# arun-sub/genomicsbench

Hardware: AMD Instinct MI355X
Metric: bsw_large_gcups (higher is better)
Workload: dtype int32

## Files before the change

genomicsbench_amd/csrc/bsw_kernels.hip:

```cpp
#include "gbx_internal.h"
#include <atomic>
#include <climits>
#include <cstdlib>

namespace gbx {
namespace {

constexpr int NEG = -(1 << 29);
constexpr int BIGJ = 1 << 20;

constexpr int NCLS = 21;
constexpr int CLS_LDS = NCLS - 1;
constexpr int NTB = 32;
constexpr int NBIN = NCLS * NTB;
constexpr int HDR = 1024;
constexpr int REG_SCORE_LIMIT = 1 << 20;

struct BswDev {
    int o_del, e_del, o_ins, e_ins, oe_del, oe_ins, zdrop, end_bonus, w, max_mat;
    uint32_t colword[5];
    int32_t col4[5];
    uint32_t row0[5];
    uint32_t row1[5];
    uint8_t remap[24];
// ... 325 lines not shown
            zm |= nz << c;
        }
        Hs[CPL] = 0;

        const int key = group_allmax<LPP>(((kl >> 5) << KB) | (j0 + (kl & 31)));
        const int m = key >> KB, mj = key & ((1 << KB) - 1);
        const int zf_l = zm ? j0 + (__builtin_ffs((int)zm) - 1) : BIGJ;
        const int zl_l = zm ? j0 + (31 - __builtin_clz(zm)) : -1;
        const int zfirst = BIGJ - group_allmax<LPP>(BIGJ - zf_l);
        const int zlast = group_allmax<LPP>(zl_l);

        const bool live = b < e;
        const int jfin = live ? e : b;
        const int hend = live ? hl : left0;
        const bool gq = jfin == qlen;
        g_i = (gq & (hend >= g_score)) ? i : g_i;
        g_score = gq ? max(g_score, hend) : g_score;
        const bool upd = (m > best) & (m != 0);
        const int dd = (i - best_i) - (mj - best_j);
        const int pen = max(__mul24(dd, e_del), __mul24(-dd, e_ins));
        const bool zbrk = (prm.zdrop > 0) & !upd & (best - m - pen > prm.zdrop);
        const bool brk = (m == 0) | zbrk;
        const int dmi = mj - i;
        off = upd ? imax3(off, dmi, -dmi) : off;
        best_i = upd ? i : best_i;
        best_j = upd ? mj : best_j;
        best = upd ? m : best;
        beg = min(zfirst, e);
        end = min(zlast + 2, qlen);
        ++i;
        done = active & (brk | (i >= tlen));
    }
}

__global__ void __launch_bounds__(64) bsw_lds_kernel(BswDev prm, BswPairs P, BswWork W, int cls)
{
    extern __shared__ int lds[];
    const int lane = threadIdx.x;
    const int first = W.base[cls * NTB];
    const int cnt = W.base[(cls + 1) * NTB] - first;
    const int32_t *order = W.order + first;
    const int e_ins = prm.e_ins, e_del = prm.e_del, oe_ins = prm.oe_ins, oe_del = prm.oe_del;

    for (int slot = blockIdx.x; slot < cnt; slot += gridDim.x) {
        const int pair = order[slot];
        const int qlen = P.len2[pair], tlen = P.len1[pair], h0 = P.h0[pair];
        const uint8_t *q = P.qer + P.idq[pair];
        const uint8_t *tp = P.ref + P.idr[pair];
        int *hd = lds, *ev = lds + (qlen + 1);
        for (int j = lane; j <= qlen; j += 64) {
            hd[j] = j == 0 ? h0 : max(h0 - oe_ins - (j - 1) * e_ins, 0);
            ev[j] = 0;
        }
        __syncthreads();
        int w;
        {
            int lim = (int)((double)(qlen * prm.max_mat + prm.end_bonus - prm.o_ins) / (double)e_ins + 1.);
            lim = max(lim, 1); w = min(prm.w, lim);
            lim = (int)((double)(qlen * prm.max_mat + prm.end_bonus - prm.o_del) / (double)e_del + 1.);
            lim = max(lim, 1); w = min(w, lim);
        }
        int best = h0, best_i = -1, best_j = -1, g_i = -1, g_score = -1, off = 0;
        int beg = 0, end = qlen;
        for (int i = 0; i < tlen; ++i) {
            const int b = max(beg, i - w);
            const int e = min(min(end, i + w + 1), qlen);
            const int left0 = b == 0 ? max(h0 - (prm.o_del + e_del * (i + 1)), 0) : 0;
            const int t = min((int)tp[i], 4);
            int fcarry = NEG;
            int left = left0;
            int m = 0, mj = -1;
            int zfirst = BIGJ, zlast = -1;
            if (left0 != 0) { zfirst = b; zlast = b; }
            for (int cb = b; cb < e; cb += 64) {
                const int j = cb + lane;
                const bool p = j < e;
                const int qc = p ? min((int)q[j], 4) : 0;
                const int s = t == 4 ? prm.col4[qc] : (int)(int8_t)(prm.colword[qc] >> (t << 3));
                const int hsv = p ? hd[j] : 0;
                const int ein = p ? ev[j] : 0;
                const int mm = (p & (hsv != 0)) ? hsv + s : 0;
                const int src = p ? max(mm - oe_ins, 0) : NEG;
                int pre = group_scan_max<64>(src + lane * e_ins);
                int fincl = pre - lane * e_ins;
                int fexcl = group_shift_up<64>(fincl, NEG, lane);
                fexcl = lane == 0 ? NEG : fexcl - 0;
                const int f = max(fexcl, fcarry - lane * e_ins);
                int h = imax3(mm, ein, f);
                h = p ? h : 0;
                const int enew = imax3(ein - e_del, mm - oe_del, 0);
                {
                    const int tot = __builtin_amdgcn_readlane(fincl, 63);
                    fcarry = max(tot, fcarry - 64 * e_ins);
                }
                int hprev = group_shift_up<64>(h, left, lane);
                hprev = lane == 0 ? left : hprev;
                left = __builtin_amdgcn_readlane(h, 63);
                if (p) { hd[j] = hprev; ev[j] = enew; }
                {
                    const int hm = group_allmax<64>(h);
                    if (hm >= m && (hm > 0 || m == 0)) {
                        const unsigned long long eq = __ballot(p && h == hm);
                        if (eq) { mj = cb + 63 - __builtin_clzll(eq); m = hm; }
                    }
                    const unsigned long long nzh = __ballot(p && h != 0);
                    const unsigned long long nze = __ballot(p && enew != 0);
                    if (nzh) {
                        zfirst = min(zfirst, cb + (int)__builtin_ctzll(nzh) + 1);
                        zlast = max(zlast, cb + 63 - (int)__builtin_clzll(nzh) + 1);
                    }
                    if (nze) {
                        zfirst = min(zfirst, cb + (int)__builtin_ctzll(nze));
                        zlast = max(zlast, cb + 63 - (int)__builtin_clzll(nze));
                    }
                }
                if (cb + 64 >= e) left = __builtin_amdgcn_readlane(h, (e - 1 - cb) & 63);
            }
            if (lane == 0) { hd[e] = b < e ? left : left0; ev[e] = 0; }
            __syncthreads();
            const int hend = b < e ? left : left0;
            const int jfin = b < e ? e : b;
            if (jfin == qlen) { g_i = g_score > hend ? g_i : i; g_score = max(g_score, hend); }
            if (m == 0) break;
            if (m > best) {
                best = m; best_i = i; best_j = mj; off = max(off, abs(mj - i));
            } else if (prm.zdrop > 0) {
                const int di = i - best_i, dj = mj - best_j;
                const int pen = di > dj ? (di - dj) * e_del : (dj - di) * e_ins;
                if (best - m - pen > prm.zdrop) break;
            }
            beg = min(zfirst, e);
            end = min(zlast + 2, qlen);
        }
        if (lane == 0) {
            gbx_bsw_result r;
            r.score = best; r.tle = best_i + 1; r.gtle = g_i + 1; r.qle = best_j + 1;
            r.gscore = g_score; r.max_off = off;
            P.out[pair] = r;
        }
        __syncthreads();
    }
}

__global__ void __launch_bounds__(256) bsw_lane_sort_kernel(BswDev prm, BswPairs P, int64_t n, BswWork W, int pass)
{
    const int64_t k = (int64_t)blockIdx.x * 256 + threadIdx.x;
    if (k >= n) return;
    const int qlen = P.len2[k], tlen = P.len1[k], h0 = P.h0[k];
    if (!lane_ok(prm.lane_on, qlen, tlen, h0, prm.max_mat) || tlen > GBX_BSW_MAX_TLEN) return;
    const int key = lane_key(qlen, h0, prm.max_mat);
    if (pass == 0) W.lrank[k] = atomicAdd(&W.lbase[key + 1], 1);
    else W.lorder[W.lbase[key] + W.lrank[k]] = (int)k;
}
__global__ void __launch_bounds__(1024) bsw_lane_scan_kernel(BswWork W)
{
    constexpr int PER = (LANE_BINS + 1023) / 1024;
    __shared__ int part[1024];
    const int tid = threadIdx.x;
    int sum = 0;
    for (int k = 0; k < PER; ++k) { const int b = tid * PER + k; if (b < LANE_BINS) sum += W.lbase[b + 1]; }
    part[tid] = sum;
    __syncthreads();
    for (int d = 1; d < 1024; d <<= 1) {
        const int add = tid >= d ? part[tid - d] : 0;
        __syncthreads();
        part[tid] += add;
        __syncthreads();
    }
    int run = part[tid] - sum;
    for (int k = 0; k < PER; ++k) {
        const int b = tid * PER + k;
        if (b < LANE_BINS) { const int c = W.lbase[b + 1]; run += c; W.lbase[b + 1] = run; }
    }
}

template <bool SYM>
__device__ __forceinline__ uint32_t lane_pair_step(uint32_t w, uint32_t qq, uint32_t rw, uint32_t rwn, int &f, int &left, uint32_t kin, uint32_t &key, int pa, int pa1,
                                                   int zero, int oe_del, int oe_ins, int e_del, int e_ins)
{
    uint32_t wn, kout;
    int hb;
    if (SYM) {
        int sa, ta, tb, ma, mb, x, ha, td, ed, ena, enb, fd, ka, kb, u, v;
        asm volatile(
            "v_perm_b32 %[sa], %[rwn], %[rw], %[qq]\n"
            "v_cmp_ne_u32_sdwa vcc, %[w], %[zero] src0_sel:BYTE_1 src1_sel:DWORD\n"
            "v_subrev_u32 %[fd], %[eins], %[f]\n"
            "v_add_u32_sdwa %[ta], sext(%[sa]), %[w] dst_sel:DWORD dst_unused:UNUSED_PAD src0_sel:BYTE_0 src1_sel:BYTE_1\n"
            "v_cndmask_b32 %[ma], 0, %[ta], vcc\n"
            "v_cmp_ne_u32_sdwa vcc, %[w], %[zero] src0_sel:BYTE_3 src1_sel:DWORD\n"
            "v_max_i32_sdwa %[x], %[ma], %[w] dst_sel:DWORD dst_unused:UNUSED_PAD src0_sel:DWORD src1_sel:BYTE_0\n"
            "v_add_u32_sdwa %[tb], sext(%[sa]), %[w] dst_sel:DWORD dst_unused:UNUSED_PAD src0_sel:BYTE_1 src1_sel:BYTE_3\n"
            "v_max_i32 %[ha], %[x], %[f]\n"
            "v_subrev_u32 %[td], %[oed], %[ma]\n"
            "v_cndmask_b32 %[mb], 0, %[tb], vcc\n"
            "v_sub_u32_sdwa %[ed], %[w], %[edel] dst_sel:DWORD dst_unused:UNUSED_PAD src0_sel:BYTE_0 src1_sel:DWORD\n"
            "v_max3_i32 %[f], %[fd], %[td], 0\n"
            "v_max3_i32 %[ena], %[ed], %[td], 0\n"
            "v_max_i32_sdwa %[x], %[mb], %[w] dst_sel:DWORD dst_unused:UNUSED_PAD src0_sel:DWORD src1_sel:BYTE_2\n"
            "v_lshl_or_b32 %[ka], %[ha], 18, %[pa]\n"
            "v_max_i32 %[hb], %[x], %[f]\n"
            "v_subrev_u32 %[td], %[oed], %[mb]\n"
            "v_subrev_u32 %[fd], %[eins], %[f]\n"
            "v_sub_u32_sdwa %[ed], %[w], %[edel] dst_sel:DWORD dst_unused:UNUSED_PAD src0_sel:BYTE_2 src1_sel:DWORD\n"
            "v_max3_i32 %[f], %[fd], %[td], 0\n"
            "v_max3_i32 %[enb], %[ed], %[td], 0\n"
            "v_lshl_or_b32 %[kb], %[hb], 18, %[pa1]\n"
            "v_lshl_or_b32 %[u], %[left], 8, %[ena]\n"
            "v_lshl_or_b32 %[v], %[ha], 8, %[enb]\n"
            "v_max3_u32 %[key], %[kin], %[ka], %[kb]\n"
            "v_lshl_or_b32 %[wn], %[v], 16, %[u]\n"
            : [sa] "=&v"(sa), [ta] "=&v"(ta), [tb] "=&v"(tb), [ma] "=&v"(ma), [mb] "=&v"(mb), [x] "=&v"(x), [ha] "=&v"(ha),
              [hb] "=&v"(hb), [td] "=&v"(td), [ed] "=&v"(ed), [ena] "=&v"(ena), [enb] "=&v"(enb), [fd] "=&v"(fd), [ka] "=&v"(ka),
              [kb] "=&v"(kb), [u] "=&v"(u), [v] "=&v"(v), [wn] "=&v"(wn), [f] "+v"(f), [key] "=v"(kout)
            : [w] "v"(w), [qq] "v"(qq), [rw] "v"(rw), [rwn] "v"(rwn), [left] "v"(left), [kin] "v"(kin), [pa] "v"(pa), [pa1] "v"(pa1), [zero] "v"(zero), [oed] "s"(oe_del),
              [edel] "s"(e_del), [eins] "s"(e_ins)
            : "vcc");
    } else {
        int sa, ta, tb, ma, mb, x, ha, td, ti, ed, ena, enb, fd, ka, kb, u, v;
        asm volatile(
            "v_perm_b32 %[sa], %[rwn], %[rw], %[qq]\n"
            "v_cmp_ne_u32_sdwa vcc, %[w], %[zero] src0_sel:BYTE_1 src1_sel:DWORD\n"
            "v_subrev_u32 %[fd], %[eins], %[f]\n"
            "v_add_u32_sdwa %[ta], sext(%[sa]), %[w] dst_sel:DWORD dst_unused:UNUSED_PAD src0_sel:BYTE_0 src1_sel:BYTE_1\n"
            "v_cndmask_b32 %[ma], 0, %[ta], vcc\n"
            "v_cmp_ne_u32_sdwa vcc, %[w], %[zero] src0_sel:BYTE_3 src1_sel:DWORD\n"
            "v_max_i32_sdwa %[x], %[ma], %[w] dst_sel:DWORD dst_unused:UNUSED_PAD src0_sel:DWORD src1_sel:BYTE_0\n"
            "v_add_u32_sdwa %[tb], sext(%[sa]), %[w] dst_sel:DWORD dst_unused:UNUSED_PAD src0_sel:BYTE_1 src1_sel:BYTE_3\n"
            "v_max_i32 %[ha], %[x], %[f]\n"
            "v_subrev_u32 %[td], %[oed], %[ma]\n"
            "v_subrev_u32 %[ti], %[oei], %[ma]\n"
            "v_cndmask_b32 %[mb], 0, %[tb], vcc\n"
            "v_sub_u32_sdwa %[ed], %[w], %[edel] dst_sel:DWORD dst_unused:UNUSED_PAD src0_sel:BYTE_0 src1_sel:DWORD\n"
            "v_max3_i32 %[f], %[fd], %[ti], 0\n"
            "v_max3_i32 %[ena], %[ed], %[td], 0\n"
            "v_max_i32_sdwa %[x], %[mb], %[w] dst_sel:DWORD dst_unused:UNUSED_PAD src0_sel:DWORD src1_sel:BYTE_2\n"
            "v_lshl_or_b32 %[ka], %[ha], 18, %[pa]\n"
            "v_max_i32 %[hb], %[x], %[f]\n"
            "v_subrev_u32 %[td], %[oed], %[mb]\n"
            "v_subrev_u32 %[ti], %[oei], %[mb]\n"
            "v_subrev_u32 %[fd], %[eins], %[f]\n"
            "v_sub_u32_sdwa %[ed], %[w], %[edel] dst_sel:DWORD dst_unused:UNUSED_PAD src0_sel:BYTE_2 src1_sel:DWORD\n"
            "v_max3_i32 %[f], %[fd], %[ti], 0\n"
            "v_max3_i32 %[enb], %[ed], %[td], 0\n"
            "v_lshl_or_b32 %[kb], %[hb], 18, %[pa1]\n"
            "v_lshl_or_b32 %[u], %[left], 8, %[ena]\n"
            "v_lshl_or_b32 %[v], %[ha], 8, %[enb]\n"
            "v_max3_u32 %[key], %[kin], %[ka], %[kb]\n"
            "v_lshl_or_b32 %[wn], %[v], 16, %[u]\n"
            : [sa] "=&v"(sa), [ta] "=&v"(ta), [tb] "=&v"(tb), [ma] "=&v"(ma), [mb] "=&v"(mb), [x] "=&v"(x), [ha] "=&v"(ha),
              [hb] "=&v"(hb), [td] "=&v"(td), [ti] "=&v"(ti), [ed] "=&v"(ed), [ena] "=&v"(ena), [enb] "=&v"(enb), [fd] "=&v"(fd), [ka] "=&v"(ka),
              [kb] "=&v"(kb), [u] "=&v"(u), [v] "=&v"(v), [wn] "=&v"(wn), [f] "+v"(f), [key] "=v"(kout)
            : [w] "v"(w), [qq] "v"(qq), [rw] "v"(rw), [rwn] "v"(rwn), [left] "v"(left), [kin] "v"(kin), [pa] "v"(pa), [pa1] "v"(pa1), [zero] "v"(zero), [oed] "s"(oe_del),
              [oei] "s"(oe_ins), [edel] "s"(e_del), [eins] "s"(e_ins)
            : "vcc");
    }
    left = hb;
    key = kout;
    return wn;
}

#ifdef GBX_BSW_LANE_STATS
__device__ unsigned long long g_bsw_lane_stats[16][4];
#endif
template <bool SYM, bool COMPACT, bool CODE4 = false, bool PACKED = false>
__global__ void __launch_bounds__(64) bsw_lane_kernel(BswDev prm, BswPairs P, BswWork W, int rlo, int rhi, int cols, int slot)
{
    extern __shared__ uint32_t lcell[];
#ifdef GBX_BSW_LANE_STATS
    __shared__ int st_rowmax[2048];
    for (int k = threadIdx.x; k < 2048; k += 64) st_rowmax[k] = 0;
    unsigned long long st_cells = 0, st_rows = 0, st_wcells = 0, st_wrows = 0;
#endif
#define LCELL(byte_addr) (*(uint32_t *)((char *)lcell + (byte_addr)))
#define LCELL16(byte_addr) (*(uint16_t *)((char *)lcell + (byte_addr)))
#define LQ8(byte_addr) (*((uint8_t *)lcell + (byte_addr)))
    const int lane = threadIdx.x;
    const int first = W.lbase[rlo << 8], count = W.lbase[(rhi + 1) << 8] - first;
    const int nchunks = (count + 63) >> 6;
    const int32_t *order = W.lorder + first;
    const int e_ins = prm.e_ins, e_del = prm.e_del, oe_ins = prm.oe_ins, oe_del = prm.oe_del;
    const int cb = lane * 4;
    constexpr int QROW = CODE4 ? 64 : 128;
    const int qb = (cols >> 1) * 256 + (CODE4 ? lane : (lane & 31) * 4 + (lane >> 5) * 2);
    auto LQREAD = [&](int a) -> uint32_t { return CODE4 ? (uint32_t)LQ8(a) : (uint32_t)LCELL16(a); };
    auto QSEL = [](uint32_t q) -> uint32_t { return CODE4 ? (((q >> 4) << 8) | (q & 15u)) : q; };
    auto QLOW = [](uint32_t q) -> uint32_t { return CODE4 ? (q & 15u) : (q & 0xffu); };
    auto cell_at = [&](int j) { return COMPACT ? (j >> 1) * 256 + cb + (j & 1) * 2 : j * 256 + cb; };
    const int tab = COMPACT ? (cols >> 1) * (256 + QROW) + 512 : (cols + 2) * 256 - 128;
    if (lane < 5) *(uint4 *)((char *)lcell + tab + lane * 16) = make_uint4(prm.row0[lane], prm.row1[lane], prm.lrow[lane], 0u);
#define LTAB(base_code) (*(const uint4 *)((const char *)lcell + tab + min((int)(base_code), 4) * 16))
    int rel0 = 0, rel1 = 2, rel2 = 256, rel3 = 258, rel4 = 512, rel5 = 514, rel6 = 768, rel7 = 770;
    asm volatile("" : "+v"(rel0), "+v"(rel1), "+v"(rel2), "+v"(rel3), "+v"(rel4), "+v"(rel5), "+v"(rel6), "+v"(rel7));
    for (;;) {
        int c = 0;
        if (lane == 0) c = atomicAdd(&W.lchunk[slot], 1);
        c = __builtin_amdgcn_readfirstlane(c);
        if (c >= nchunks) break;
        const int hi_ = count - (c << 6), idx = hi_ - 64 + lane;
        const bool have = idx >= 0;
        const int pair = order[have ? idx : 0];
        const int qlen = P.len2[pair], tlen = P.len1[pair], h0 = P.h0[pair];
        const int64_t qo = P.idq[pair], to = P.idr[pair];
        const uint8_t *q = P.qer + (PACKED ? 0 : qo);
        const uint8_t *t = P.ref + (PACKED ? 0 : to);
        auto qpiece = [&](int j) -> uint4 {
            uint4 r;
            if (!PACKED) { __builtin_memcpy(&r, q + j, 16); return r; }
            const int64_t o = qo + j;
            const uint8_t *b = q + (o >> 1);
            uint64_t v;
            __builtin_memcpy(&v, b, 8);
            if (o & 1) v = (v >> 4) | ((uint64_t)b[8] << 60);
            auto spread = [](unsigned h) -> unsigned { return (h & 0xfu) | ((h & 0xf0u) << 4) | ((h & 0xf00u) << 8) | ((h & 0xf000u) << 12); };
            const unsigned lo = (unsigned)v, hi = (unsigned)(v >> 32);
            r.x = spread(lo & 0xffffu); r.y = spread(lo >> 16); r.z = spread(hi & 0xffffu); r.w = spread(hi >> 16);
            return r;
        };
        auto tbase = [&](int i) -> int {
            if (!PACKED) return t[i];
            const int64_t o = to + i;
            return (t[o >> 1] >> ((int)(o & 1) * 4)) & 15;
        };
        {
            uint4 wq = qpiece(0);
// ... 370 lines not shown
        int best = h0, best_i = -1, best_j = -1, g_i = -1, g_score = -1, off = 0;
        int beg = 0, end = qlen;
        bool running = true;
        uint2 mrow = s_tab[min((int)t[0], 4)], mnext = s_tab[min((int)t[1], 4)];
        int tb2 = t[2];
        const uint8_t *tp = t + 3;
        int hrow = h0 - prm.o_del - e_del;
        int imw = -w, ipw = w + 1;
        for (int i = 0;; ++i) {
            if (!__any(running)) break;
            const uint32_t rw = mrow.x, rwn = mrow.y;
            mrow = mnext;
            mnext = s_tab[min(tb2, 4)];
            tb2 = running ? (int)*tp : 0;
            tp += running ? 1 : 0;
            beg = max(beg, imw);
            end = min(min(end, ipw), qlen);
            ++imw; ++ipw;
            int left = beg == 0 ? max(hrow, 0) : 0;
            hrow -= e_del;
            const int bb = running ? beg : OUT, ee = running ? end : OUT;
            const int sp0 = bb >> 1, sq = max((ee >> 1) - 1, 0);
            const uint32_t touch = running ? bit_span(bb >> 3, min(ee >> 3, NB - 1)) : 0u;
            const uint32_t whole = running ? bit_span((bb + 7) >> 3, min((ee >> 3) - 1, NB - 1)) : ~0u;
            auto blk = [](int pp) { return pp < 4 * NB ? 1u << (pp >> 2) : 0u; };
            const uint32_t probe = running ? blk(sp0) | blk(sp0 + 1) | blk(sq) | blk(sq + 1) : 0u;
            const uint32_t touch_w = wave_bits<false>(touch), whole_w = wave_bits<true>(whole), probe_w = wave_bits<false>(probe);
            int vzero = 0;
            asm volatile("" : "+v"(vzero));
            int f = 0;
            uint32_t key = 0;
#pragma unroll
            for (int b = 0; b < NB; ++b) {
                if (!((touch_w >> b) & 1u)) continue;
                const uint32_t sa0 = __builtin_amdgcn_perm(rwn, rw, qs[2 * b]);
                const uint32_t sa1 = 2 * b + 1 < NQ ? __builtin_amdgcn_perm(rwn, rw, qs[2 * b + 1]) : 0u;
                uint32_t kt = (uint32_t)vzero;
                if ((whole_w >> b) & 1u) {
                    cell[4 * b] = reg_pair_step<SYM, false, 0>(cell[4 * b], sa0, f, left, kt, vzero, oe_del, oe_ins, e_del, e_ins);
                    if (4 * b + 1 < NCP) cell[4 * b + 1] = reg_pair_step<SYM, true, 2>(cell[4 * b + 1], sa0, f, left, kt, vzero, oe_del, oe_ins, e_del, e_ins);
                    if (4 * b + 2 < NCP) cell[4 * b + 2] = reg_pair_step<SYM, false, 4>(cell[4 * b + 2], sa1, f, left, kt, vzero, oe_del, oe_ins, e_del, e_ins);
                    if (4 * b + 3 < NCP) cell[4 * b + 3] = reg_pair_step<SYM, true, 6>(cell[4 * b + 3], sa1, f, left, kt, vzero, oe_del, oe_ins, e_del, e_ins);
                } else {
                    int lb = bb - 8 * b, le = ee - 8 * b;
                    asm volatile("" : "+v"(lb), "+v"(le));
                    reg_pair_masked<SYM, false, 0>(cell[4 * b], sa0, lb, le, f, left, kt, vzero, oe_del, oe_ins, e_del, e_ins);
                    if (4 * b + 1 < NCP) reg_pair_masked<SYM, true, 2>(cell[4 * b + 1], sa0, lb, le, f, left, kt, vzero, oe_del, oe_ins, e_del, e_ins);
                    if (4 * b + 2 < NCP) reg_pair_masked<SYM, false, 4>(cell[4 * b + 2], sa1, lb, le, f, left, kt, vzero, oe_del, oe_ins, e_del, e_ins);
                    if (4 * b + 3 < NCP) reg_pair_masked<SYM, true, 6>(cell[4 * b + 3], sa1, lb, le, f, left, kt, vzero, oe_del, oe_ins, e_del, e_ins);
                }
                key = max(key, kt + (uint32_t)(8 * b));
            }
            uint32_t sb0 = 0, sb1 = 0, se0 = 0, se1 = 0;
#pragma unroll
            for (int b = 0; b < NB; ++b) {
                if (!((probe_w >> b) & 1u)) continue;
                int db = sp0 - 4 * b, de = sq - 4 * b;
                asm volatile("" : "+v"(db), "+v"(de));
#pragma unroll
                for (int m = 0; m < 4 && 4 * b + m < NCP; ++m) {
                    const uint32_t cv = cell[4 * b + m];
                    sb0 = db == m ? cv : sb0;
                    sb1 = db == m - 1 ? cv : sb1;
                    se0 = de == m ? cv : se0;
                    se1 = de == m - 1 ? cv : se1;
                }
            }
            if (running) {
                const int jfin = beg < end ? end : beg;
                if (jfin == qlen) {
                    if (!(g_score > left)) g_i = i;
                    g_score = max(g_score, left);
                }
                const int row_best = (int)(key >> 18), row_arg = (int)(key & 0x3ffffu);
                bool stop = row_best == 0;
                if (!stop) {
                    if (row_best > best) {
                        best = row_best; best_i = i; best_j = row_arg;
                        off = max(off, abs(row_arg - i));
                    } else if (prm.zdrop > 0) {
                        const int di = i - best_i, dj = row_arg - best_j;
                        stop = di > dj ? best - row_best - (di - dj) * e_del > prm.zdrop : best - row_best - (dj - di) * e_ins > prm.zdrop;
                    }
                }
                if (!stop) {
                    int k = (sb1 >> 16) ? 3 : 4;
                    k = (sb1 & 0xffffu) ? 2 : k;
                    k = (sb0 >> 16) ? 1 : k;
                    k = (sb0 & 0xffffu) && !(beg & 1) ? 0 : k;
                    int j = 2 * sp0 + k;
                    const int khi = end - 2 * sq;
                    int ke = (se0 & 0xffffu) ? 0 : -1;
                    ke = (se0 >> 16) && khi >= 1 ? 1 : ke;
                    ke = (se1 & 0xffffu) && khi >= 2 ? 2 : ke;
                    ke = (se1 >> 16) && khi >= 3 ? 3 : ke;
                    uint32_t nz[NW];
                    if (k == 4 || ke < 0) {
#pragma unroll
                        for (int u = 0; u < NW; ++u) nz[u] = 0u;
#pragma unroll
                        for (int p = 0; p < NCP; ++p) {
                            const uint32_t two = ((cell[p] & 0xffffu) ? 1u : 0u) | ((cell[p] >> 16) ? 2u : 0u);
                            nz[p >> 4] |= two << ((2 * p) & 31);
                        }
                    }
                    if (k == 4) {
                        int jn = end;
#pragma unroll
                        for (int u = NW - 1; u >= 0; --u) {
                            const uint32_t m = nz[u] & bits_from(j - 32 * u) & ~bits_from(end - 32 * u);
                            jn = m ? 32 * u + __builtin_ctz(m) : jn;
                        }
                        j = jn;
                    }
                    j = min(j, end);
                    const int nbeg = beg < end ? j : beg;
                    j = 2 * sq + ke;
                    if (ke < 0 && 2 * sq > nbeg) {
                        int jl = nbeg - 1;
#pragma unroll
                        for (int u = 0; u < NW; ++u) {
                            const uint32_t m = nz[u] & bits_from(nbeg - 32 * u) & ~bits_from(j + 1 - 32 * u);
                            jl = m ? 32 * u + 31 - __builtin_clz(m) : jl;
                        }
                        j = jl;
                    }
                    j = max(j, nbeg - 1);
                    j = nbeg > end ? end : j;
                    beg = nbeg;
                    end = min(j + 2, qlen);
                }
                running = !stop && i + 1 < tlen;
            }
        }
        gbx_bsw_result r;
        r.score = best; r.tle = best_i + 1; r.gtle = g_i + 1; r.qle = best_j + 1; r.gscore = g_score; r.max_off = off;
        if (have) P.out[pair] = r;
    }
}

typedef void (*RowsFn)(BswDev, BswPairs, BswWork, int);
struct RowKernel { int lpp, cpl; RowsFn fn[2]; std::atomic<int> bpc[2]; const char *name; };
#define GBX_ROW_KERNEL(L, C) { L, C, { bsw_rows_kernel<L, C, false>, bsw_rows_kernel<L, C, true> }, { 0, 0 }, "bsw_rows_" #L "x" #C }
RowKernel row_kernels[] = {
    GBX_ROW_KERNEL(2, 4),  GBX_ROW_KERNEL(2, 8),  GBX_ROW_KERNEL(2, 12), GBX_ROW_KERNEL(2, 16), GBX_ROW_KERNEL(2, 20), GBX_ROW_KERNEL(2, 24),
    GBX_ROW_KERNEL(4, 14), GBX_ROW_KERNEL(4, 16), GBX_ROW_KERNEL(4, 18), GBX_ROW_KERNEL(4, 20), GBX_ROW_KERNEL(4, 22), GBX_ROW_KERNEL(4, 24),
    GBX_ROW_KERNEL(8, 13), GBX_ROW_KERNEL(8, 14), GBX_ROW_KERNEL(8, 15), GBX_ROW_KERNEL(8, 16),
    GBX_ROW_KERNEL(16, 10), GBX_ROW_KERNEL(16, 12), GBX_ROW_KERNEL(16, 16), GBX_ROW_KERNEL(64, 16),
    GBX_ROW_KERNEL(16, 8), GBX_ROW_KERNEL(64, 3), GBX_ROW_KERNEL(64, 4),
};
#undef GBX_ROW_KERNEL
static_assert(sizeof(row_kernels) / sizeof(row_kernels[0]) >= NCLS - 1, "one row kernel per register class");

constexpr uint8_t CLASS_REMAP[3][NCLS] = {
    {0, 1, 2, 3, 4, 5, 6, 7, 8, 9, 10, 11, 12, 13, 14, 15, 16, 17, 18, 19, 20},
    {3, 3, 3, 3, 7, 7, 7, 7, 11, 11, 11, 11, 15, 15, 15, 15, 18, 18, 18, 19, 20},
    {15, 15, 15, 15, 15, 15, 15, 15, 15, 15, 15, 15, 15, 15, 15, 15, 18, 18, 18, 19, 20},
};
int class_mode_for(int64_t n)
{
    const char *e = getenv("GBX_BSW_CLASSMODE");
    if (e && *e >= '0' && *e <= '2') return *e - '0';
    return n < 32768 ? 2 : n < 250000 ? 1 : 0;
}

RowKernel *find_row_kernel(int lpp, int cpl)
{
    for (RowKernel &k : row_kernels)
        if (k.lpp == lpp && k.cpl == cpl) return &k;
    return nullptr;
}

typedef void (*LaneFn)(BswDev, BswPairs, BswWork, int, int, int, int);
enum { LANE_COMPACT = 0, LANE_COMPACT4 = 1, LANE_WIDE = 2 };
#define GBX_LANE_KERNEL(COMPACT, CODE4, PACKED) { bsw_lane_kernel<false, COMPACT, CODE4, PACKED>, bsw_lane_kernel<true, COMPACT, CODE4, PACKED> }
const LaneFn lane_kernels[2][3][2] = {
    { GBX_LANE_KERNEL(true, false, false), GBX_LANE_KERNEL(true, true, false), GBX_LANE_KERNEL(false, false, false) },
    { GBX_LANE_KERNEL(true, false, true),  GBX_LANE_KERNEL(true, true, true),  GBX_LANE_KERNEL(false, false, true) },
};
#undef GBX_LANE_KERNEL

int resident_blocks(std::atomic<int> &cache, const void *fn, int threads, int fallback, int cap)
{
    int bpc = cache.load(std::memory_order_relaxed);
    if (bpc) return bpc;
    if (hipOccupancyMaxActiveBlocksPerMultiprocessor(&bpc, fn, threads, 0) != hipSuccess || bpc < 1) { (void)hipGetLastError(); bpc = fallback; }
    bpc = bpc > cap ? cap : bpc;
    cache.store(bpc, std::memory_order_relaxed);
    return bpc;
}

bool switched_off(const char *name) { const char *e = getenv(name); return e && atoi(e) == 0; }

int make_dev_params(const gbx_bsw_params *p, BswDev *d)
{
    if (p->e_del < 1 || p->e_ins < 1 || p->o_del < 0 || p->o_ins < 0 || p->e_del > 4096 || p->e_ins > 4096 ||
        p->o_del > (1 << 16) || p->o_ins > (1 << 16) || p->w < 0) {
        set_error("bsw: gap penalties must satisfy 0<=o<=65536, 1<=e<=4096, w>=0");
        return GBX_ERR_ARG;
    }
    d->o_del = p->o_del; d->e_del = p->e_del; d->o_ins = p->o_ins; d->e_ins = p->e_ins;
    d->oe_del = p->o_del + p->e_del; d->oe_ins = p->o_ins + p->e_ins;
    d->zdrop = p->zdrop; d->end_bonus = p->end_bonus; d->w = p->w;
    int mx = 0;
    for (int k = 0; k < 25; ++k) mx = p->mat[k] > mx ? p->mat[k] : mx;
    d->max_mat = mx;
    for (int q = 0; q < 5; ++q) {
        uint32_t wv = 0;
        for (int t = 0; t < 4; ++t) wv |= (uint32_t)(uint8_t)p->mat[t * 5 + q] << (8 * t);
        d->colword[q] = wv;
        d->col4[q] = p->mat[4 * 5 + q];
    }
    for (int t = 0; t < 5; ++t) {
        uint32_t wv = 0;
        for (int q = 0; q < 4; ++q) wv |= (uint32_t)(uint8_t)p->mat[t * 5 + q] << (8 * q);
        d->row0[t] = wv;
        d->row1[t] = (uint32_t)(uint8_t)p->mat[t * 5 + 4];
    }
    d->lane_on = 0;
    bool fits6 = true;
    for (int k = 0; k < 25; ++k) fits6 = fits6 && p->mat[k] >= -32 && p->mat[k] <= 31;
    for (int t = 0; t < 5; ++t) {
        uint32_t wv = 0;
        for (int q = 0; q < 5; ++q) wv |= ((uint32_t)p->mat[t * 5 + q] & 63u) << (6 * q);
        d->lrow[t] = wv;
    }
    if (fits6 && p->o_del + p->e_del < LANE_SCORE_LIMIT && p->o_ins + p->e_ins < LANE_SCORE_LIMIT) d->lane_on = -1;
    return GBX_OK;
}

}

constexpr int64_t WS_LANE = (int64_t)(LANE_BINS + 64) + 64;
size_t bsw_workspace_bytes(int64_t n)
{
    return (size_t)(WS_HDR + 4 * (n > 0 ? n : 0) + WS_LANE) * sizeof(int32_t);
}

constexpr int UNPACK_ROUNDS = 4;
__device__ inline unsigned spread4(unsigned h) { return (h & 0xfu) | ((h & 0xf0u) << 4) | ((h & 0xf00u) << 8) | ((h & 0xf000u) << 12); }
__global__ void __launch_bounds__(256) bsw_unpack4_kernel(const uint8_t *__restrict__ packed, uint8_t *__restrict__ out, int64_t lo, int64_t hi)
{
    const int64_t base = lo + (int64_t)blockIdx.x * (256 * 16 * UNPACK_ROUNDS) + threadIdx.x * 16;
    const bool aligned = (((uintptr_t)(packed + (base >> 1)) & 7) == 0) && (((uintptr_t)(out + base) & 15) == 0);
    if (aligned && base + (int64_t)(UNPACK_ROUNDS - 1) * 4096 + 16 <= hi) {
        uint2 v[UNPACK_ROUNDS];
#pragma unroll
        for (int r = 0; r < UNPACK_ROUNDS; ++r) v[r] = *(const uint2 *)(packed + ((base + r * 4096) >> 1));
#pragma unroll
        for (int r = 0; r < UNPACK_ROUNDS; ++r) {
            uint4 q;
            q.x = spread4(v[r].x & 0xffffu); q.y = spread4(v[r].x >> 16); q.z = spread4(v[r].y & 0xffffu); q.w = spread4(v[r].y >> 16);
            *(uint4 *)(out + base + r * 4096) = q;
        }
        return;
    }
    for (int r = 0; r < UNPACK_ROUNDS; ++r) {
        const int64_t o = base + r * 4096;
        if (o >= hi) return;
        if (aligned && o + 16 <= hi) {
            const uint2 v = *(const uint2 *)(packed + (o >> 1));
            uint4 q;
            q.x = spread4(v.x & 0xffffu); q.y = spread4(v.x >> 16); q.z = spread4(v.y & 0xffffu); q.w = spread4(v.y >> 16);
            *(uint4 *)(out + o) = q;
        } else {
            for (int64_t k = o; k < o + 16 && k < hi; ++k) out[k] = (uint8_t)((packed[k >> 1] >> ((k & 1) * 4)) & 0xf);
        }
    }
}

int bsw_unpack4(const uint8_t *d_packed, uint8_t *d_out, int64_t lo, int64_t hi, hipStream_t s)
{
    if (hi <= lo) return GBX_OK;
    const int64_t per_block = 256 * 16 * UNPACK_ROUNDS;
    Stage st("bsw_unpack4", s);
    hipLaunchKernelGGL(bsw_unpack4_kernel, dim3((unsigned)((hi - lo + per_block - 1) / per_block)), dim3(256), 0, s, d_packed, d_out, lo, hi);
    GBX_HIP(hipGetLastError());
    return GBX_OK;
}

int bsw_launch_direct(const gbx_bsw_params *p, int64_t n, int max_qlen,
                      const uint8_t *d_ref, const uint8_t *d_qer, const int64_t *d_idr, const int64_t *d_idq,
                      const int32_t *d_len1, const int32_t *d_len2, const int32_t *d_h0, gbx_bsw_result *d_out, hipStream_t s)
{
    if (n <= 0) return GBX_OK;
    BswDev dev;
    int rc = make_dev_params(p, &dev);
    if (rc) return rc;
    for (int c = 0; c < NCLS; ++c) dev.remap[c] = (uint8_t)c;
    BswPairs P = {d_ref, d_qer, d_idr, d_idq, d_len1, d_len2, d_h0, d_out};
    BswWork W = {nullptr, nullptr, nullptr, nullptr, nullptr, nullptr, nullptr, nullptr, nullptr, nullptr};
    dev.lane_on = 0;
    if (max_qlen > 256) { set_error("bsw: direct launch needs queries of at most 256"); return GBX_ERR_ARG; }
    const int cols = max_qlen + 1;
    int lpp = 16, cpl = cols <= 128 ? 8 : cols <= 160 ? 10 : cols <= 192 ? 12 : 16;
    if (n < 4096) { lpp = 64; cpl = cols <= 192 ? 3 : 4; }
    if (const char *e = getenv("GBX_BSW_DIRECT_SHAPE")) {
        int l = 0, c = 0;
        if (sscanf(e, "%dx%d", &l, &c) == 2 && l * c > max_qlen && find_row_kernel(l, c)) { lpp = l; cpl = c; }
    }
    RowKernel *k = find_row_kernel(lpp, cpl);
    if (!k) { set_error("bsw: no %dx%d row kernel", lpp, cpl); return GBX_ERR_UNSUPPORTED; }
    const bool sym = dev.oe_ins == dev.oe_del;
    const int gpb = 256 / lpp;
    const int blocks = (int)((n + gpb - 1) / gpb);
    Stage st(k->name, s);
    hipLaunchKernelGGL(k->fn[sym], dim3(blocks), dim3(256), 0, s, dev, P, W, -(int)n);
    GBX_HIP(hipGetLastError());
    return GBX_OK;
}

static std::atomic<long long> g_lane_reg_launches{0};

static bool lane_wanted(int64_t n)
{
    const char *lane_env = getenv("GBX_BSW_LANE");
    const int64_t lane_min = getenv("GBX_BSW_LANE_MIN") ? atoll(getenv("GBX_BSW_LANE_MIN")) : 262144;
    return lane_env ? atoi(lane_env) != 0 : n >= lane_min;
}

int bsw_lane_rule(const gbx_bsw_params *p, int64_t n, BswLaneRule *r)
{
    BswDev dev;
    const int rc = make_dev_params(p, &dev);
    if (rc) return rc;
    r->on = dev.lane_on && lane_wanted(n) ? 1 : 0;
    r->max_mat = dev.max_mat > 0 ? dev.max_mat : 0;
    r->qmax = LANE_QMAX;
    r->limit = LANE_SCORE_LIMIT;
    return GBX_OK;
}

struct BswCall {
    BswDev dev; BswPairs P; BswWork W;
    int64_t n;
    int mode, cus;
    bool sym;
    hipStream_t s; SideStreams *ss; hipEvent_t *join_events; const BswChunkPrep *prep;
    bool ahead;
    bool no_rows;
    bool packed_lanes;
    int phase;
    hipStream_t s_cls;
    hipEvent_t ev_pre, ev_aux;
};

static int plan_call(BswCall &c)
{
    const BswChunkPrep *prep = c.prep;
    static const bool prep_off = switched_off("GBX_BSW_PREP");
    c.ahead = prep && prep->uploaded && c.join_events && !prep_off;
    c.s_cls = c.ahead ? c.ss->pre[0] : c.s;
    c.no_rows = c.dev.lane_on && prep && prep->rows_pairs == 0 && !switched_off("GBX_BSW_SKIP_ROWS");
    c.packed_lanes = c.no_rows && prep->ref_packed && !switched_off("GBX_BSW_PACKED_LANES");
    c.phase = prep ? prep->phase : 0;
    if (c.phase && !(c.ahead && c.packed_lanes && prep->ev_pre && prep->ev_aux)) {
        if (c.phase == 1) return 1;
        set_error("bsw: the kernels of a chunk whose preparing passes were not queued");
        return GBX_ERR_ARG;
    }
    c.ev_pre = c.phase ? prep->ev_pre : c.ss->ev_pre;
    c.ev_aux = c.phase ? prep->ev_aux : c.ss->ev_aux;
    if (c.packed_lanes) { c.P.ref = prep->ref_packed; c.P.qer = prep->qer_packed; c.P.packed = 1; }
    return GBX_OK;
}

static int queue_prepare(BswCall &c)
{
    const BswChunkPrep *prep = c.prep;
    SideStreams *ss = c.ss;
    const int64_t n = c.n;
    int rc;
    if (c.ahead) {
        GBX_HIP(hipStreamWaitEvent(ss->pre[0], prep->uploaded, 0));
        GBX_HIP(hipStreamWaitEvent(ss->pre[1], prep->uploaded, 0));
    }
    if (!c.packed_lanes && prep && prep->ref_packed) {
        const int64_t from_r = prep->unp_r ? *prep->unp_r : prep->lo_r, from_q = prep->unp_q ? *prep->unp_q : prep->lo_q;
        if ((rc = bsw_unpack4(prep->ref_packed, prep->ref_bytes, from_r, prep->hi_r, c.s_cls)) ||
            (rc = bsw_unpack4(prep->qer_packed, prep->qer_bytes, from_q, prep->hi_q, c.s_cls)))
            return rc;
        if (prep->unp_r && prep->hi_r > *prep->unp_r) *prep->unp_r = prep->hi_r;
        if (prep->unp_q && prep->hi_q > *prep->unp_q) *prep->unp_q = prep->hi_q;
    }
    GBX_HIP(hipMemsetAsync(c.W.counts, 0, WS_HDR * sizeof(int32_t), c.s_cls));
    if (c.dev.lane_on) {
        hipStream_t so;
        if (c.ahead) {
            so = ss->pre[1];
            GBX_HIP(hipMemsetAsync(c.W.lbase, 0, (size_t)WS_LANE * sizeof(int32_t), so));
        } else {
            GBX_HIP(hipMemsetAsync(c.W.lbase, 0, (size_t)WS_LANE * sizeof(int32_t), c.s));
            if ((rc = ss->fork(c.s))) return rc;
            so = ss->side[SideStreams::N - 1];
        }
        Stage st("bsw_lane_sort", so);
        const int sblocks = (int)((n + 255) / 256);
        hipLaunchKernelGGL(bsw_lane_sort_kernel, dim3(sblocks), dim3(256), 0, so, c.dev, c.P, n, c.W, 0);
        hipLaunchKernelGGL(bsw_lane_scan_kernel, dim3(1), dim3(1024), 0, so, c.W);
        hipLaunchKernelGGL(bsw_lane_sort_kernel, dim3(sblocks), dim3(256), 0, so, c.dev, c.P, n, c.W, 1);
        GBX_HIP(hipEventRecord(c.ev_aux, so));
    }
    const int cblocks = (int)((n + CLS_THREADS - 1) / CLS_THREADS);
    {
        Stage st("bsw_classify", c.s_cls);
        hipLaunchKernelGGL(bsw_classify_kernel, dim3(cblocks), dim3(CLS_THREADS), 0, c.s_cls, c.dev, c.P, n, c.W, 0);
        hipLaunchKernelGGL(bsw_scan_kernel, dim3(1), dim3(HDR), 0, c.s_cls, c.W);
        hipLaunchKernelGGL(bsw_classify_kernel, dim3(cblocks), dim3(CLS_THREADS), 0, c.s_cls, c.dev, c.P, n, c.W, 1);
    }
    if (c.ahead) GBX_HIP(hipEventRecord(c.ev_pre, c.s_cls));
    GBX_HIP(hipGetLastError());
    return GBX_OK;
}

static int kernel_streams_wait(const BswCall &c, hipEvent_t ev, int n_side = SideStreams::N)
{
    GBX_HIP(hipStreamWaitEvent(c.s, ev, 0));
    for (int k = 0; k < n_side; ++k) GBX_HIP(hipStreamWaitEvent(c.ss->side[k], ev, 0));
    return GBX_OK;
}

static void launch_row_classes(BswCall &c)
{
    const int nk = c.join_events ? 3 : 4;
    int launched = 0;
    for (int cls = 0; cls < NCLS - 1; ++cls) {
        if (CLASS_REMAP[c.mode][cls] != cls) continue;
        const int sk = (c.mode ? launched++ : cls) % nk;
        hipStream_t sc = c.dev.lane_on || sk == 0 ? c.s : c.ss->side[sk - 1];
        RowKernel &k = row_kernels[cls];
        const int bpc = resident_blocks(k.bpc[c.sym], (const void *)k.fn[c.sym], 256, 2, 8);
        const int gpb = 256 / k.lpp;
        const int64_t want = (c.n + gpb - 1) / gpb, cap = (int64_t)c.cus * bpc;
        Stage st(k.name, sc);
        hipLaunchKernelGGL(k.fn[c.sym], dim3((int)(want < cap ? want : cap)), dim3(256), 0, sc, c.dev, c.P, c.W, cls);
    }
}

static void launch_lane_reg(const BswCall &c, hipStream_t sc, int64_t want, int rlo, int rhi, int slot)
{
    static_assert(LANE_RANGE_HI[0][2] == 99, "bsw_lane_reg_kernel instance");
    typedef void (*LaneRegFn)(BswDev, BswPairs, BswWork, int, int, int);
    static const LaneRegFn reg_fn[2] = {bsw_lane_reg_kernel<false, 99>, bsw_lane_reg_kernel<true, 99>};
    static std::atomic<int> reg_bpc[2];
    const int64_t cap = (int64_t)c.cus * resident_blocks(reg_bpc[c.sym], (const void *)reg_fn[c.sym], 64, 8, INT_MAX);
    hipLaunchKernelGGL(reg_fn[c.sym], dim3((unsigned)(want < cap ? want : cap)), dim3(64), 0, sc, c.dev, c.P, c.W, rlo, rhi, slot);
    g_lane_reg_launches.fetch_add(1, std::memory_order_relaxed);
}

static void launch_lanes(const BswCall &c)
{
    static const char *names[2][LANE_NRANGE] = {{"bsw_lane_c47", "bsw_lane_c79", "bsw_lane_c99", "bsw_lane_c135", "bsw_lane_c159"},
                                                {"bsw_lane_w39", "bsw_lane_w79", "bsw_lane_w103", "bsw_lane_w127", "bsw_lane_w159"}};
    const int64_t want = (c.n + 63) / 64;
    for (int fmt = 1; fmt >= 0; --fmt) {
        for (int r = LANE_NRANGE - 1; r >= 0; --r) {
            const int qlo = r ? LANE_RANGE_HI[fmt][r - 1] + 1 : 1, qhi = LANE_RANGE_HI[fmt][r];
            const int cols = (qhi + 3) & ~1;
            const int kind = fmt ? LANE_WIDE : qhi > 99 ? LANE_COMPACT4 : LANE_COMPACT;
            const size_t lds = fmt ? (size_t)(cols + 2) * 256 : (size_t)(cols / 2) * (kind == LANE_COMPACT4 ? 320 : 384) + 640;
            const int fit = (int)((size_t)160 * 1024 / lds), per_cu = fit > 16 ? 16 : fit;
            const int sk = (LANE_NRANGE - 1 - r) & 3;
            hipStream_t sc = sk == 0 ? c.s : c.ss->side[sk - 1];
            const int64_t cap = (int64_t)c.cus * per_cu;
            const int rlo = fmt * (LANE_QMAX + 1) + qlo, rhi = fmt * (LANE_QMAX + 1) + qhi, slot = fmt * LANE_NRANGE + r;
            Stage st(names[fmt][r], sc);
            if (fmt == 0 && !c.P.packed && qhi == 99 && !switched_off("GBX_BSW_LANE_REG")) { launch_lane_reg(c, sc, want, rlo, rhi, slot); continue; }
            hipLaunchKernelGGL(lane_kernels[c.P.packed][kind][c.sym], dim3((unsigned)(want < cap ? want : cap)), dim3(64), lds, sc,
                               c.dev, c.P, c.W, rlo, rhi, cols, slot);
        }
    }
}

static int launch_lds(const BswCall &c)
{
    const size_t lds_bytes = (size_t)(GBX_BSW_MAX_QLEN + 1) * 2 * sizeof(int);
    static std::atomic<uint64_t> attr_set[2];
    int cur = 0;
    GBX_HIP(hipGetDevice(&cur));
    const uint64_t bit = (uint64_t)1 << (cur & 63);
    if (cur >= 128 || !(attr_set[cur >> 6].load(std::memory_order_acquire) & bit)) {
        GBX_HIP(hipFuncSetAttribute((const void *)bsw_lds_kernel, hipFuncAttributeMaxDynamicSharedMemorySize, (int)lds_bytes));
        if (cur < 128) attr_set[cur >> 6].fetch_or(bit, std::memory_order_release);
    }
    const int blocks = (int)(c.n < (int64_t)c.cus * 2 ? c.n : (int64_t)c.cus * 2);
    Stage st("bsw_lds", c.s);
    hipLaunchKernelGGL(bsw_lds_kernel, dim3(blocks), dim3(64), lds_bytes, c.s, c.dev, c.P, c.W, CLS_LDS);
    return GBX_OK;
}

int bsw_launch(const gbx_bsw_params *p, int64_t n,
               const uint8_t *d_ref, const uint8_t *d_qer,
               const int64_t *d_idr, const int64_t *d_idq,
               const int32_t *d_len1, const int32_t *d_len2, const int32_t *d_h0,
               gbx_bsw_result *d_out, void *d_work, size_t work_bytes, hipStream_t s, hipEvent_t *join_events,
               const BswChunkPrep *prep)
{
    if (n == 0) return GBX_OK;
    if (n > 0x7fffffffLL - 1024) { set_error("bsw: more than 2^31 pairs in one call"); return GBX_ERR_UNSUPPORTED; }
    if (work_bytes < bsw_workspace_bytes(n)) { set_error("bsw: workspace too small"); return GBX_ERR_ARG; }
    BswCall c;
    int rc = make_dev_params(p, &c.dev);
    if (rc) return rc;
    c.n = n; c.mode = class_mode_for(n); c.cus = 256;
    for (int k = 0; k < NCLS; ++k) c.dev.remap[k] = CLASS_REMAP[c.mode][k];
    c.P = {d_ref, d_qer, d_idr, d_idq, d_len1, d_len2, d_h0, d_out};
    int32_t *wi = (int32_t *)d_work, *wl = wi + WS_HDR + 4 * n;
    c.W = {wi, wi + HDR, wi + 2 * HDR, wi + 3 * HDR, wi + WS_HDR, wi + WS_HDR + n, wl, wi + WS_HDR + 3 * n, wi + WS_HDR + 2 * n, wl + LANE_BINS + 64};
    c.dev.lane_on = c.dev.lane_on && lane_wanted(n) ? 1 : 0;
    c.sym = c.dev.oe_ins == c.dev.oe_del;
    c.s = s; c.join_events = join_events; c.prep = prep;
    if ((rc = side_streams(&c.ss))) return rc;
    std::unique_lock<std::mutex> side_lock(c.ss->mu);
    if ((rc = plan_call(c))) return rc;
    if (c.phase != 2) {
        if ((rc = queue_prepare(c))) return rc;
        if (c.phase == 1) return GBX_OK;
    }
    if (c.ahead) {
        if ((rc = kernel_streams_wait(c, c.ev_pre))) return rc;
        if (c.phase == 2 && (rc = kernel_streams_wait(c, prep->uploaded))) return rc;
    }
    int dev_id = 0;
    (void)hipGetDevice(&dev_id);
    (void)hipDeviceGetAttribute(&c.cus, hipDeviceAttributeMultiprocessorCount, dev_id);
    if (!c.dev.lane_on && !c.ahead && (rc = c.ss->fork(s))) return rc;
    if (!c.no_rows) launch_row_classes(c);
    if (c.dev.lane_on) {
        if ((rc = kernel_streams_wait(c, c.ev_aux, c.ahead ? SideStreams::N : SideStreams::N - 1))) return rc;
        launch_lanes(c);
    }
    if (!join_events && (rc = c.ss->join(s))) return rc;
    if (!c.no_rows && (rc = launch_lds(c))) return rc;
    if (join_events) {
        GBX_HIP(hipEventRecord(join_events[0], s));
        for (int k = 0; k < SideStreams::N; ++k) GBX_HIP(hipEventRecord(join_events[1 + k], c.ss->side[k]));
    }
    GBX_HIP(hipGetLastError());
    return GBX_OK;
}

}

extern "C" long long gbx_debug_bsw_lane_reg_launches(void)
{
    return gbx::g_lane_reg_launches.load(std::memory_order_relaxed);
}

#ifdef GBX_BSW_LANE_STATS
extern "C" int gbx_debug_bsw_lane_stats(unsigned long long *out, int reset)
{
    if (hipMemcpyFromSymbol(out, HIP_SYMBOL(gbx::g_bsw_lane_stats), sizeof(unsigned long long) * 64) != hipSuccess) return -1;
    if (reset) { unsigned long long z[64] = {0}; if (hipMemcpyToSymbol(HIP_SYMBOL(gbx::g_bsw_lane_stats), z, sizeof(z)) != hipSuccess) return -1; }
    return 0;
}
#endif
```

Before: 2532.

## Overlap row-class kernels with lane kernels on side streams; faster lane scan

```diff
diff --git a/genomicsbench_amd/csrc/bsw_kernels.hip b/genomicsbench_amd/csrc/bsw_kernels.hip
--- a/genomicsbench_amd/csrc/bsw_kernels.hip
+++ b/genomicsbench_amd/csrc/bsw_kernels.hip
@@ -501,25 +501,66 @@
     if (pass == 0) W.lrank[k] = atomicAdd(&W.lbase[key + 1], 1);
     else W.lorder[W.lbase[key] + W.lrank[k]] = (int)k;
 }
+__device__ inline int wave_scan_add(int x)
+{
+    x += dpp<0x111>(0, x);
+    x += dpp<0x112>(0, x);
+    x += dpp<0x114>(0, x);
+    x += dpp<0x118>(0, x);
+    x += dpp<0x142, 0xa>(0, x);
+    x += dpp<0x143, 0xc>(0, x);
+    return x;
+}
 __global__ void __launch_bounds__(1024) bsw_lane_scan_kernel(BswWork W)
 {
-    constexpr int PER = (LANE_BINS + 1023) / 1024;
-    __shared__ int part[1024];
-    const int tid = threadIdx.x;
-    int sum = 0;
-    for (int k = 0; k < PER; ++k) { const int b = tid * PER + k; if (b < LANE_BINS) sum += W.lbase[b + 1]; }
-    part[tid] = sum;
+    constexpr int NE = LANE_BINS + 1, TILE = 4096, TILES = (NE + TILE - 1) / TILE, NW = 1024 / 64;
+    constexpr int PER0 = (TILES * NW + 63) / 64;
+    __shared__ int wsum[PER0 * 64];
+    const int tid = threadIdx.x, lane = tid & 63, wave = tid >> 6;
+    int32_t *lb = W.lbase;
+    const bool vec = ((uintptr_t)lb & 15) == 0;
+    auto load4 = [&](int b) {
+        if (vec && b + 3 < NE) return *(const int4 *)(lb + b);
+        return make_int4(b < NE ? lb[b] : 0, b + 1 < NE ? lb[b + 1] : 0, b + 2 < NE ? lb[b + 2] : 0, b + 3 < NE ? lb[b + 3] : 0);
+    };
+    int pre[TILES];
+#pragma unroll
+    for (int t = 0; t < TILES; ++t) {
+        const int4 v = load4(t * TILE + tid * 4);
+        pre[t] = v.x + v.y + v.z + v.w;
+    }
+    for (int k = tid; k < PER0 * 64; k += 1024) wsum[k] = 0;
     __syncthreads();
-    for (int d = 1; d < 1024; d <<= 1) {
-        const int add = tid >= d ? part[tid - d] : 0;
-        __syncthreads();
-        part[tid] += add;
-        __syncthreads();
-    }
-    int run = part[tid] - sum;
-    for (int k = 0; k < PER; ++k) {
-        const int b = tid * PER + k;
-        if (b < LANE_BINS) { const int c = W.lbase[b + 1]; run += c; W.lbase[b + 1] = run; }
+#pragma unroll
+    for (int t = 0; t < TILES; ++t) {
+        const int incl = wave_scan_add(pre[t]);
+        if (lane == 63) wsum[t * NW + wave] = incl;
+        pre[t] = incl - pre[t];
+    }
+    __syncthreads();
+    if (wave == 0) {
+        int s[PER0], sum = 0;
+#pragma unroll
+        for (int k = 0; k < PER0; ++k) { s[k] = wsum[lane * PER0 + k]; sum += s[k]; }
+        int run = wave_scan_add(sum) - sum;
+#pragma unroll
+        for (int k = 0; k < PER0; ++k) { wsum[lane * PER0 + k] = run; run += s[k]; }
+    }
+    __syncthreads();
+#pragma unroll
+    for (int t = 0; t < TILES; ++t) {
+        const int b = t * TILE + tid * 4;
+        const int4 v = load4(b);
+        int4 o;
+        o.x = wsum[t * NW + wave] + pre[t] + v.x;
+        o.y = o.x + v.y; o.z = o.y + v.z; o.w = o.z + v.w;
+        if (vec && b + 3 < NE) *(int4 *)(lb + b) = o;
+        else {
+            if (b < NE) lb[b] = o.x;
+            if (b + 1 < NE) lb[b + 1] = o.y;
+            if (b + 2 < NE) lb[b + 2] = o.z;
+            if (b + 3 < NE) lb[b + 3] = o.w;
+        }
     }
 }
 
@@ -1196,15 +1237,18 @@
 #undef GBX_ROW_KERNEL
 static_assert(sizeof(row_kernels) / sizeof(row_kernels[0]) >= NCLS - 1, "one row kernel per register class");
 
-constexpr uint8_t CLASS_REMAP[3][NCLS] = {
+constexpr int LANE_CLASS_MODE = 3;
+constexpr uint8_t CLASS_REMAP[4][NCLS] = {
     {0, 1, 2, 3, 4, 5, 6, 7, 8, 9, 10, 11, 12, 13, 14, 15, 16, 17, 18, 19, 20},
     {3, 3, 3, 3, 7, 7, 7, 7, 11, 11, 11, 11, 15, 15, 15, 15, 18, 18, 18, 19, 20},
     {15, 15, 15, 15, 15, 15, 15, 15, 15, 15, 15, 15, 15, 15, 15, 15, 18, 18, 18, 19, 20},
+    {15, 15, 15, 15, 15, 15, 15, 15, 15, 15, 15, 15, 15, 15, 15, 15, 16, 17, 18, 19, 20},
 };
-int class_mode_for(int64_t n)
+int class_mode_for(int64_t n, bool lane_on)
 {
     const char *e = getenv("GBX_BSW_CLASSMODE");
     if (e && *e >= '0' && *e <= '2') return *e - '0';
+    if (lane_on) return LANE_CLASS_MODE;
     return n < 32768 ? 2 : n < 250000 ? 1 : 0;
 }
 
@@ -1452,7 +1496,7 @@
         hipLaunchKernelGGL(bsw_scan_kernel, dim3(1), dim3(HDR), 0, c.s_cls, c.W);
         hipLaunchKernelGGL(bsw_classify_kernel, dim3(cblocks), dim3(CLS_THREADS), 0, c.s_cls, c.dev, c.P, n, c.W, 1);
     }
-    if (c.ahead) GBX_HIP(hipEventRecord(c.ev_pre, c.s_cls));
+    if (c.ahead || (c.dev.lane_on && !c.no_rows)) GBX_HIP(hipEventRecord(c.ev_pre, c.s_cls));
     GBX_HIP(hipGetLastError());
     return GBX_OK;
 }
@@ -1471,7 +1515,7 @@
     for (int cls = 0; cls < NCLS - 1; ++cls) {
         if (CLASS_REMAP[c.mode][cls] != cls) continue;
         const int sk = (c.mode ? launched++ : cls) % nk;
-        hipStream_t sc = c.dev.lane_on || sk == 0 ? c.s : c.ss->side[sk - 1];
+        hipStream_t sc = sk == 0 ? c.s : c.ss->side[sk - 1];
         RowKernel &k = row_kernels[cls];
         const int bpc = resident_blocks(k.bpc[c.sym], (const void *)k.fn[c.sym], 256, 2, 8);
         const int gpb = 256 / k.lpp;
@@ -1546,12 +1590,13 @@
     BswCall c;
     int rc = make_dev_params(p, &c.dev);
     if (rc) return rc;
-    c.n = n; c.mode = class_mode_for(n); c.cus = 256;
-    for (int k = 0; k < NCLS; ++k) c.dev.remap[k] = CLASS_REMAP[c.mode][k];
+    c.n = n; c.cus = 256;
     c.P = {d_ref, d_qer, d_idr, d_idq, d_len1, d_len2, d_h0, d_out};
     int32_t *wi = (int32_t *)d_work, *wl = wi + WS_HDR + 4 * n;
     c.W = {wi, wi + HDR, wi + 2 * HDR, wi + 3 * HDR, wi + WS_HDR, wi + WS_HDR + n, wl, wi + WS_HDR + 3 * n, wi + WS_HDR + 2 * n, wl + LANE_BINS + 64};
     c.dev.lane_on = c.dev.lane_on && lane_wanted(n) ? 1 : 0;
+    c.mode = class_mode_for(n, c.dev.lane_on);
+    for (int k = 0; k < NCLS; ++k) c.dev.remap[k] = CLASS_REMAP[c.mode][k];
     c.sym = c.dev.oe_ins == c.dev.oe_del;
     c.s = s; c.join_events = join_events; c.prep = prep;
     if ((rc = side_streams(&c.ss))) return rc;
@@ -1569,11 +1614,13 @@
     (void)hipGetDevice(&dev_id);
     (void)hipDeviceGetAttribute(&c.cus, hipDeviceAttributeMultiprocessorCount, dev_id);
     if (!c.dev.lane_on && !c.ahead && (rc = c.ss->fork(s))) return rc;
-    if (!c.no_rows) launch_row_classes(c);
     if (c.dev.lane_on) {
         if ((rc = kernel_streams_wait(c, c.ev_aux, c.ahead ? SideStreams::N : SideStreams::N - 1))) return rc;
         launch_lanes(c);
-    }
+        if (!c.no_rows && !c.ahead)
+            for (int k = 0; k < SideStreams::N; ++k) GBX_HIP(hipStreamWaitEvent(c.ss->side[k], c.ev_pre, 0));
+    }
+    if (!c.no_rows) launch_row_classes(c);
     if (!join_events && (rc = c.ss->join(s))) return rc;
     if (!c.no_rows && (rc = launch_lds(c))) return rc;
     if (join_events) {
```

Result: slower. 2490 (-1.7%).
